# IXarea/LittleGAN

Hardware: AMD Instinct MI355X
Metric: 128x128 CelebA-shaped images/sec (G+D+Adj step) (higher is better)
Workload: dtype bf16; 1 GPU; C3: 128x128x3 synthetic CelebA, batch 256/GPU, bf16 MFMA conv/transposed-conv + Adjuster branch; global_batch=256, per_gpu_batch=256, image=128, cond_dim=40, parallelism=dp1, launch=eager launches

## Files before the change

### littlegan_amd/csrc/norm.hip

```cpp
#include "lg_common.h"
#include "philox.h"

#define LG_IN_EPS 1e-3f
#define LG_NSTAT 8

namespace {

constexpr int CHUNK = 4096;
constexpr int EW_UNR = 4;

__global__ __launch_bounds__(256) void stats_partial_kernel(const float* __restrict__ x, double* __restrict__ partial,
                                                            long long L, int nchunk, int pre_leaky, float alpha,
                                                            __bf16* __restrict__ x16out) {
  const int n = blockIdx.y, ch = blockIdx.x;
  const long long base = (long long)n * L + (long long)ch * CHUNK;
  const long long lim = L - (long long)ch * CHUNK;
  __shared__ double sred[32];
  f32x4 v[4];
  double s = 0.0;
  int cnt = 0;
#pragma unroll
  for (int q = 0; q < 4; ++q) {
    const int e = (q * 256 + threadIdx.x) * 4;
    v[q] = f32x4{0.f, 0.f, 0.f, 0.f};
// ... 183 lines not shown
   const long long lim = L - c0;
#pragma unroll
   for (int q = 0; q < 4; ++q) {
    const int e = (q * 256 + threadIdx.x) * 4;
    if (e < lim) {
      const f32x4 xv = *reinterpret_cast<const f32x4*>(x + base + e);
      const f32x4 gv = load_g4(g, base + e, g16);
      float q1 = 0.f, q2 = 0.f;
      float dm[4];
      if constexpr (DROP) drop_mult4(dc, (unsigned long long)(base + e) >> 2, dm);
#pragma unroll
      for (int k = 0; k < 4; ++k) {
        float xx = xv[k];
        if (pre_leaky) xx = lg_leaky(xx, alpha);
        const float c = (xx - mu) - mul;
        float dz = gv[k];
        if constexpr (DROP) dz = dz * dm[k];
        if (post_leaky) dz = (a * c + b > 0.f) ? dz : alpha * dz;
        q1 += dz;
        q2 += dz * c;
      }
      s1 += (double)q1;
      s2 += (double)q2;
    }
   }
  }
  double red[2] = {s1, s2};
  lg_block_sum_d<2>(red, sred);
  if (threadIdx.x == 0) {
    double* o = partial + ((long long)n * nchunk + blockIdx.x) * 2;
    o[0] = red[0]; o[1] = red[1];
  }
}

__global__ __launch_bounds__(256) void bwd_partial_kernel(const float* __restrict__ x, const void* __restrict__ g, int g16,
                                                          const float* __restrict__ stats, double* __restrict__ partial,
                                                          long long L, int nchunk, int pre_leaky, int post_leaky,
                                                          float alpha) {
  bwd_partial_body<false>(x, g, g16, stats, partial, L, nchunk, pre_leaky, post_leaky, alpha, DropK{}, Geo{blockDim.x, gridDim.x, gridDim.y});
}
__global__ __launch_bounds__(256) void bwd_partial_drop_kernel(const float* __restrict__ x, const void* __restrict__ g, int g16,
                                                               const float* __restrict__ stats, double* __restrict__ partial,
                                                               long long L, int nchunk, float alpha, DropK dk) {
  bwd_partial_body<true>(x, g, g16, stats, partial, L, nchunk, 0, 1, alpha, dk, Geo{blockDim.x, gridDim.x, gridDim.y});
}

__global__ __launch_bounds__(64) void bwd_final_kernel(const double* __restrict__ partial, const float* __restrict__ stats,
                                                       float* __restrict__ bstats, double* __restrict__ gsum,
                                                       long long L, int nchunk) {
  const int n = blockIdx.x, lane = threadIdx.x;
  const double* p = partial + (long long)n * nchunk * 2;
  double s1 = 0.0, s2 = 0.0;
  for (int i = lane; i < nchunk; i += 64) { s1 += p[i * 2]; s2 += p[i * 2 + 1]; }
  s1 = lg_wave_sum_d(s1); s2 = lg_wave_sum_d(s2);
  if (lane == 0) {
    const double sigma = (double)stats[(long long)n * LG_NSTAT + 1], s = sigma + (double)LG_IN_EPS;
    const double m1 = s1 / (double)L, m2 = s2 / (double)L / (s * sigma);
    const float m1h = (float)m1, m2h = (float)m2;
    bstats[n * 4] = m1h; bstats[n * 4 + 1] = m2h;
    bstats[n * 4 + 2] = (float)(m1 - (double)m1h); bstats[n * 4 + 3] = (float)(m2 - (double)m2h);
    gsum[n * 2] = s2 / s;
    gsum[n * 2 + 1] = s1;
  }
}

__global__ __launch_bounds__(64) void bwd_coef_kernel(const double* __restrict__ partial, const float* __restrict__ stats,
                                                      float* __restrict__ coef, long long L, int nchunk) {
  const int n = blockIdx.x, lane = threadIdx.x;
  const double* p = partial + (long long)n * nchunk * 2;
  double s1 = 0.0, s2 = 0.0;
  for (int i = lane; i < nchunk; i += 64) { s1 += p[i * 2]; s2 += p[i * 2 + 1]; }
  s1 = lg_wave_sum_d(s1); s2 = lg_wave_sum_d(s2);
  if (lane == 0) {
    const float* sp = stats + (long long)n * LG_NSTAT;
    const double sigma = (double)sp[1], s = sigma + (double)LG_IN_EPS;
    const double m1 = s1 / (double)L, m2 = s2 / (double)L / (s * sigma);
    const float m1h = (float)m1, m2h = (float)m2;
    float* o = coef + (long long)n * 8;
    o[0] = sp[0]; o[1] = sp[4]; o[2] = sp[2]; o[3] = sp[3];
    o[4] = m1h; o[5] = m2h; o[6] = (float)(m1 - (double)m1h); o[7] = (float)(m2 - (double)m2h);
  }
}

__global__ __launch_bounds__(256) void bwd_affine_grad_kernel(const double* __restrict__ gsum, float* __restrict__ dgamma,
                                                              float* __restrict__ dbeta, int B, int accumulate) {
  __shared__ double sg[256], sb[256];
  double g = 0.0, b = 0.0;
  for (int i = threadIdx.x; i < B; i += 256) { g += gsum[i * 2]; b += gsum[i * 2 + 1]; }
  sg[threadIdx.x] = g; sb[threadIdx.x] = b;
  __syncthreads();
  for (int o = 128; o > 0; o >>= 1) {
    if (threadIdx.x < o) { sg[threadIdx.x] += sg[threadIdx.x + o]; sb[threadIdx.x] += sb[threadIdx.x + o]; }
    __syncthreads();
  }
  if (threadIdx.x == 0) {
    dgamma[0] = (accumulate ? dgamma[0] : 0.f) + (float)sg[0];
    dbeta[0] = (accumulate ? dbeta[0] : 0.f) + (float)sb[0];
  }
}

template <bool DB, bool DROP>
__device__ __forceinline__ void bwd_apply_body(const float* __restrict__ x, const void* __restrict__ g, int g16,
                                               const float* __restrict__ stats, const float* __restrict__ bstats,
                                               float* __restrict__ dx, __bf16* __restrict__ dx16, long long L4,
                                               long long total4, int pre_leaky, int post_leaky, float alpha,
                                               float* __restrict__ colpart, int C4, const DropK& dk, const Geo ge) {
  const DropCtx dc = drop_begin<DROP>(dk);
  constexpr int UNR = DB ? 1 : EW_UNR;
  const unsigned stride = ge.gdx * ge.bdx * UNR, tot = (unsigned)total4, l4 = (unsigned)L4;
  f32x4 csum = {0.f, 0.f, 0.f, 0.f};
  const unsigned rb = blockIdx.x;
  const int ntrip = (int)(((unsigned long long)tot + stride - 1) / stride);
  for (int tr = 0; tr < ntrip; ++tr) {
   const unsigned long long i0l = (unsigned long long)tr * stride + rb * ge.bdx * UNR + threadIdx.x;
   if (i0l >= tot) continue;
   const unsigned i0 = (unsigned)i0l;
   f32x4 xs[UNR], gs[UNR];
#pragma unroll
   for (int u = 0; u < UNR; ++u) {
     const unsigned i = i0 + u * 256;
     if (i < tot) {
       xs[u] = lg_ld<NT_LOAD>(reinterpret_cast<const f32x4*>(x + (long long)i * 4));
       gs[u] = load_g4<NT_LOAD>(g, (long long)i * 4, g16);
     }
   }
#pragma unroll
   for (int u = 0; u < UNR; ++u) {
    const unsigned i = i0 + u * 256;
    if (i >= tot) break;
    const int n = (int)(i / l4);
    const float* sp = stats + (long long)n * LG_NSTAT;
    const float mu = sp[0], a = sp[2], b = sp[3], mul = sp[4];
    const float m1 = bstats[n * 4], m2 = bstats[n * 4 + 1], m1l = bstats[n * 4 + 2], m2l = bstats[n * 4 + 3];
    const f32x4 xv = xs[u], gv = gs[u];
    f32x4 o;
    float dm[4];
    if constexpr (DROP) drop_mult4(dc, i, dm);
#pragma unroll
    for (int k = 0; k < 4; ++k) {
      float xx = xv[k];
      if (pre_leaky) xx = lg_leaky(xx, alpha);
      const float c = (xx - mu) - mul;
      float dz = gv[k];
      if constexpr (DROP) dz = dz * dm[k];
      if (post_leaky) dz = (a * c + b > 0.f) ? dz : alpha * dz;
      float d = a * ((((dz - m1) - m1l) - c * m2) - c * m2l);
      if (pre_leaky) d = (xv[k] > 0.f) ? d : alpha * d;
      o[k] = d;
    }
    if (dx) *reinterpret_cast<f32x4*>(dx + (long long)i * 4) = o;
    if (dx16) {
      bf16x4 w;
      w[0] = (__bf16)o[0]; w[1] = (__bf16)o[1]; w[2] = (__bf16)o[2]; w[3] = (__bf16)o[3];
      *reinterpret_cast<bf16x4*>(dx16 + (long long)i * 4) = w;
    }
    if constexpr (DB) csum += o;
   }
  }
  if constexpr (DB) {
    __shared__ f32x4 sacc[256];
    sacc[threadIdx.x] = csum;
    __syncthreads();
    const int q = threadIdx.x;
    if (q < C4) {
      const int base = (int)(((long long)rb * 256) % C4);
      f32x4 t = {0.f, 0.f, 0.f, 0.f};
      for (int k = (q - base + C4) % C4; k < 256; k += C4) t += sacc[k];
      *reinterpret_cast<f32x4*>(colpart + ((long long)rb * C4 + q) * 4) = t;
    }
  }
}
template <bool DB>
__global__ __launch_bounds__(256) void bwd_apply_kernel(const float* __restrict__ x, const void* __restrict__ g, int g16,
                                                        const float* __restrict__ stats, const float* __restrict__ bstats,
                                                        float* __restrict__ dx, __bf16* __restrict__ dx16, long long L4,
                                                        long long total4, int pre_leaky, int post_leaky, float alpha,
                                                        float* __restrict__ colpart, int C4) {
  bwd_apply_body<DB, false>(x, g, g16, stats, bstats, dx, dx16, L4, total4, pre_leaky, post_leaky, alpha, colpart, C4, DropK{}, Geo{blockDim.x, gridDim.x, gridDim.y});
}
template <bool DB>
__global__ __launch_bounds__(256) void bwd_apply_drop_kernel(const float* __restrict__ x, const void* __restrict__ g, int g16,
// ... 253 lines not shown
                                                 long long total8, int pre_leaky, int post_leaky, float alpha,
                                                 float* __restrict__ colpart, int C8, const DropK& dk, const Geo ge) {
  const DropCtx dc = drop_begin<DROP>(dk);
  constexpr int UNR = DB ? DB_UNR : EW8_UNR;
  const unsigned tot = (unsigned)total8, l8 = (unsigned)L8;
  const unsigned ustep = DB ? ge.gdx * ge.bdx : 256u;
  const unsigned stride = DB ? ge.gdx * ge.bdx * UNR : ge.gdx * ge.bdx * UNR;
  const unsigned rb = ge.gdx - 1 - blockIdx.x;
  const unsigned first = DB ? rb * ge.bdx + threadIdx.x : rb * ge.bdx * UNR + threadIdx.x;
  f32x8 csum;
  csum.lo = f32x4{0.f, 0.f, 0.f, 0.f}; csum.hi = f32x4{0.f, 0.f, 0.f, 0.f};
  const int ntrip = (int)(((unsigned long long)tot + stride - 1) / stride);
  for (int tr = 0; tr < ntrip; ++tr) {
    const unsigned long long i0l = (unsigned long long)(ntrip - 1 - tr) * stride + first;
    if (i0l >= tot) continue;
    const unsigned i0 = (unsigned)i0l;
    f32x8 xs[UNR], gs[UNR];
#pragma unroll
    for (int u = 0; u < UNR; ++u) {
      const unsigned i = i0 + u * ustep;
      if (i < tot) { xs[u] = load8<true, NT_LOAD>(x, i); gs[u] = load8<G16, NT_LOAD>(g, i); }
    }
#pragma unroll
    for (int u = 0; u < UNR; ++u) {
      const unsigned i = i0 + u * ustep;
      if (i >= tot) break;
      const int n = (int)(i / l8);
      const float* sp = stats + (long long)n * LG_NSTAT;
      const float mu = sp[0], a = sp[2], b = sp[3], mul = sp[4];
      const float m1 = bstats[n * 4], m2 = bstats[n * 4 + 1], m1l = bstats[n * 4 + 2], m2l = bstats[n * 4 + 3];
      f32x8 o;
      float dm[8];
      if constexpr (DROP) drop_mult8(dc, i, dm);
#pragma unroll
      for (int k = 0; k < 8; ++k) {
        const float x0 = k < 4 ? xs[u].lo[k & 3] : xs[u].hi[k & 3];
        float xx = x0;
        if (pre_leaky) xx = lg_leaky(xx, alpha);
        const float c = (xx - mu) - mul;
        float dz = k < 4 ? gs[u].lo[k & 3] : gs[u].hi[k & 3];
        if constexpr (DROP) dz = dz * dm[k];
        if (post_leaky) dz = (a * c + b > 0.f) ? dz : alpha * dz;
        float d = a * ((((dz - m1) - m1l) - c * m2) - c * m2l);
        if (pre_leaky) d = (x0 > 0.f) ? d : alpha * d;
        if (k < 4) o.lo[k & 3] = d; else o.hi[k & 3] = d;
      }
      if (dx) store8_f32(dx, i, o);
      if (dx16) store8_bf16(dx16, i, o);
      if constexpr (DB) { csum.lo += o.lo; csum.hi += o.hi; }
    }
  }
  if constexpr (DB) {
    __shared__ f32x4 sacc[512];
    sacc[2 * threadIdx.x] = csum.lo; sacc[2 * threadIdx.x + 1] = csum.hi;
    __syncthreads();
    const int q = threadIdx.x;
    if (q < C8) {
      const int base = (int)(((long long)rb * 256) % C8);
      f32x4 tl = {0.f, 0.f, 0.f, 0.f}, th = {0.f, 0.f, 0.f, 0.f};
      for (int k = (q - base + C8) % C8; k < 256; k += C8) { tl += sacc[2 * k]; th += sacc[2 * k + 1]; }
      *reinterpret_cast<f32x4*>(colpart + ((long long)rb * C8 + q) * 8) = tl;
      *reinterpret_cast<f32x4*>(colpart + ((long long)rb * C8 + q) * 8 + 4) = th;
    }
  }
}

template <bool DB, bool G16>
__global__ __launch_bounds__(256) void bwd_apply16_kernel(const __bf16* __restrict__ x, const void* __restrict__ g,
                                                          const float* __restrict__ stats, const float* __restrict__ bstats,
                                                          float* __restrict__ dx, __bf16* __restrict__ dx16, long long L8,
                                                          long long total8, int pre_leaky, int post_leaky, float alpha,
                                                          float* __restrict__ colpart, int C8) {
  bwd_apply16_body<DB, G16, false>(x, g, stats, bstats, dx, dx16, L8, total8, pre_leaky, post_leaky, alpha, colpart, C8, DropK{}, Geo{blockDim.x, gridDim.x, gridDim.y});
}
template <bool DB, bool G16>
__global__ __launch_bounds__(256) void bwd_apply16_drop_kernel(const __bf16* __restrict__ x, const void* __restrict__ g,
                                                               const float* __restrict__ stats, const float* __restrict__ bstats,
                                                               float* __restrict__ dx, __bf16* __restrict__ dx16, long long L8,
                                                               long long total8, float alpha, float* __restrict__ colpart, int C8,
                                                               DropK dk) {
  bwd_apply16_body<DB, G16, true>(x, g, stats, bstats, dx, dx16, L8, total8, 0, 1, alpha, colpart, C8, dk, Geo{blockDim.x, gridDim.x, gridDim.y});
}

__global__ __launch_bounds__(256) void dropout_mask_kernel(unsigned char* __restrict__ keep, long long total8, DropK dk) {
  const DropCtx dc = drop_begin<true>(dk);
  for (long long i = (long long)blockIdx.x * 256 + threadIdx.x; i < total8; i += (long long)gridDim.x * 256) {
    float dm[8];
    drop_mult8(dc, (unsigned long long)i, dm);
    unsigned lo = 0, hi = 0;
#pragma unroll
    for (int k = 0; k < 4; ++k) { lo |= (dm[k] != 0.f ? 1u : 0u) << (8 * k); hi |= (dm[4 + k] != 0.f ? 1u : 0u) << (8 * k); }
    *reinterpret_cast<unsigned long long*>(keep + i * 8) = (unsigned long long)lo | ((unsigned long long)hi << 32);
  }
}

__global__ __launch_bounds__(1024) void colsum_final_kernel(const float* __restrict__ partial, float* __restrict__ db, int nb,
                                                            int C, int accumulate) {
  __shared__ float sr[64][17];
  const int cl = threadIdx.x & 15, gq = threadIdx.x >> 4;
  const int c = blockIdx.x * 16 + cl;
  float s = 0.f;
  if (c < C) {
    int k = gq;
    for (; k + 192 < nb; k += 256) {
      const float a = partial[(long long)k * C + c], b = partial[(long long)(k + 64) * C + c];
      const float e = partial[(long long)(k + 128) * C + c], f = partial[(long long)(k + 192) * C + c];
      s += (a + b) + (e + f);
    }
    for (; k < nb; k += 64) s += partial[(long long)k * C + c];
  }
  sr[gq][cl] = s;
  __syncthreads();
  if (gq == 0 && c < C) {
    float t = 0.f;
#pragma unroll
    for (int q = 0; q < 64; q += 4) t += (sr[q][cl] + sr[q + 1][cl]) + (sr[q + 2][cl] + sr[q + 3][cl]);
    db[c] = (accumulate ? db[c] : 0.f) + t;
  }
}

constexpr long long EW_MAX_BLOCKS = 8192;
extern "C" int lg_device_cus(void);
#define LG_RESIDENT_BLOCKS(kern)                                                                                       \
  ([]() -> long long {                                                                                                 \
    static long long r = 0;                                                                                            \
    if (!r) {                                                                                                          \
      int per_cu = 0;                                                                                                  \
      if (hipOccupancyMaxActiveBlocksPerMultiprocessor(&per_cu, kern, 256, 0) != hipSuccess || per_cu < 1) per_cu = 8; \
      r = (long long)per_cu * lg_device_cus();                                                                         \
    }                                                                                                                  \
    return r;                                                                                                          \
  }())
inline long long fit_rounds(long long nb, long long resident, long long hard, int unit) {
  if (nb > hard) nb = hard;
  if (nb > resident) nb = nb / resident * resident;
  nb = nb / unit * unit;
  return nb < unit ? unit : nb;
}
inline int nchunks(long long L) { return (int)((L + CHUNK - 1) / CHUNK); }
inline int ew_blocks(long long total4) {
  long long b = (total4 + 256 * EW_UNR - 1) / (256 * EW_UNR);
  return (int)(b < EW_MAX_BLOCKS ? (b > 0 ? b : 1) : EW_MAX_BLOCKS);
}
inline size_t part_bytes(int B, long long L) { return ((size_t)B * nchunks(L) * 3 * sizeof(double) + 255) / 256 * 256; }
inline size_t bst_bytes(int B) { return ((size_t)B * 4 * sizeof(float) + 255) / 256 * 256; }

int drop_args(const char* who, const long long* key, int call, int level, int r0, int B, long long L, float rate, DropK* dk) {
  LG_CHECK_ARG(key, "%s: null pointer (dropout key)", who);
  LG_CHECK_ARG(L > 0 && L % 8 == 0, "%s: dropout needs L %% 8 == 0 (one Philox block per 8 elements), got L=%lld", who, L);
  LG_CHECK_ARG(rate >= 0.f && rate < 1.f, "%s: dropout rate %g outside [0, 1)", who, (double)rate);
  LG_CHECK_ARG(call >= 0 && call <= 3, "%s: dropout call slot %d outside 0..3", who, call);
  LG_CHECK_ARG(level >= 1 && level <= 4, "%s: dropout level %d outside 1..4", who, level);
  LG_CHECK_ARG(r0 >= 0 && B > 0 && ((unsigned long long)r0 + (unsigned long long)B) * (unsigned long long)(L / 8) <= (1ull << 32),
               "%s: first row %d + %d rows of %lld elements leave the level's counter window", who, r0, B, L);
  const long long T = llrint((double)rate * 65536.0);
  LG_CHECK_ARG(T < 65536, "%s: dropout rate %g rounds to 1", who, (double)rate);
  dk->key = reinterpret_cast<const unsigned long long*>(key);
  dk->base = ((unsigned long long)call << 34) + ((unsigned long long)(level - 1) << 32) + (unsigned long long)r0 * (unsigned long long)(L / 8);
  dk->T = (unsigned)T;
  dk->scale = 65536.f / (float)(65536 - T);
  return LG_OK;
}

}

extern "C" int lg_instnorm_stats_stride(void) { return LG_NSTAT; }

extern "C" size_t lg_instnorm_workspace_bytes(int B, long long L) {
  const size_t gs = ((size_t)B * 2 * sizeof(double) + 255) / 256 * 256;
  return part_bytes(B, L) + bst_bytes(B) + gs;
}

extern "C" int lg_instnorm_leaky_stats_z16(const float* x, float* stats, const float* gamma, const float* beta,
                                           void* workspace, size_t ws_bytes, int B, long long L, int pre_leaky,
                                           float alpha, void* x16_out, void* stream);
extern "C" int lg_instnorm_leaky_stats(const float* x, float* stats, const float* gamma, const float* beta,
                                       void* workspace, size_t ws_bytes, int B, long long L, int pre_leaky,
                                       float alpha, void* stream) {
  return lg_instnorm_leaky_stats_z16(x, stats, gamma, beta, workspace, ws_bytes, B, L, pre_leaky, alpha, nullptr, stream);
}
extern "C" int lg_instnorm_leaky_stats_z16(const float* x, float* stats, const float* gamma, const float* beta,
                                           void* workspace, size_t ws_bytes, int B, long long L, int pre_leaky,
                                           float alpha, void* x16_out, void* stream) {
  LG_CHECK_ARG(x && stats && gamma && beta && workspace, "lg_instnorm_leaky_stats: null pointer");
  LG_CHECK_ARG(B > 0 && B <= 65535 && L > 0 && L % 4 == 0, "lg_instnorm_leaky_stats: bad shape B=%d L=%lld", B, L);
  LG_CHECK_ARG(ws_bytes >= lg_instnorm_workspace_bytes(B, L), "lg_instnorm_leaky_stats: workspace too small");
  hipStream_t st = (hipStream_t)stream;
  const int nc = nchunks(L);
  hipLaunchKernelGGL(stats_partial_kernel, dim3(nc, B), dim3(256), 0, st, x, (double*)workspace, L, nc, pre_leaky, alpha,
                     (__bf16*)x16_out);
  LG_CHECK_LAUNCH("lg_instnorm_leaky_stats(partial)");
  hipLaunchKernelGGL(stats_final_kernel, dim3(B), dim3(64), 0, st, (const double*)workspace, stats, gamma, beta, nc);
  LG_CHECK_LAUNCH("lg_instnorm_leaky_stats(final)");
  return LG_OK;
}

extern "C" int lg_instnorm_stats_finalize(const void* partials, int nparts, float* stats, const float* gamma,
                                          const float* beta, int B, void* stream) {
  LG_CHECK_ARG(partials && stats && gamma && beta && nparts > 0 && B > 0, "lg_instnorm_stats_finalize: bad arguments");
  hipLaunchKernelGGL(stats_final_kernel, dim3(B), dim3(64), 0, (hipStream_t)stream, (const double*)partials, stats, gamma,
                     beta, nparts);
  LG_CHECK_LAUNCH("lg_instnorm_stats_finalize");
  return LG_OK;
}

static int apply_impl(const float* x, const float* stats, const float* skip, float* y, void* y16, int B, long long L, int pre_leaky,
                      int post_leaky, float alpha, const DropK* dk, void* stream) {
  LG_CHECK_ARG(x && stats && (y || y16), "lg_instnorm_leaky_apply: null pointer");
  LG_CHECK_ARG(B > 0 && L > 0 && L % 4 == 0 && (long long)B * L / 4 < (1LL << 31), "lg_instnorm_leaky_apply: bad shape B=%d L=%lld", B, L);
  const long long total4 = (long long)B * L / 4;
  if (dk) {
    hipLaunchKernelGGL(apply_drop_kernel, dim3((int)fit_rounds(ew_blocks(total4), LG_RESIDENT_BLOCKS(apply_drop_kernel), EW_MAX_BLOCKS, 1)), dim3(256), 0,
                       (hipStream_t)stream, x, stats, y, (__bf16*)y16, L / 4, total4, alpha, *dk);
    LG_CHECK_LAUNCH("lg_instnorm_leaky_apply_drop");
    return LG_OK;
  }
  hipLaunchKernelGGL(apply_kernel, dim3((int)fit_rounds(ew_blocks(total4), LG_RESIDENT_BLOCKS(apply_kernel), EW_MAX_BLOCKS, 1)), dim3(256), 0, (hipStream_t)stream, x, stats, skip, y,
                     (__bf16*)y16, L / 4, total4, pre_leaky, post_leaky, alpha);
  LG_CHECK_LAUNCH("lg_instnorm_leaky_apply");
  return LG_OK;
}
extern "C" int lg_instnorm_leaky_apply(const float* x, const float* stats, const float* skip, float* y, void* y16, int B,
                                       long long L, int pre_leaky, int post_leaky, float alpha, void* stream) {
  return apply_impl(x, stats, skip, y, y16, B, L, pre_leaky, post_leaky, alpha, nullptr, stream);
}
extern "C" int lg_instnorm_leaky_apply_drop(const float* x, const float* stats, float* y, void* y16, int B, long long L, float alpha,
                                            const long long* key, int call, int level, int r0, float rate, void* stream) {
  DropK dk;
  if (int rc = drop_args("lg_instnorm_leaky_apply_drop", key, call, level, r0, B, L, rate, &dk)) return rc;
  return apply_impl(x, stats, nullptr, y, y16, B, L, 0, 1, alpha, &dk, stream);
}

constexpr int DB_MAX_BLOCKS = 2046;

extern "C" size_t lg_instnorm_bwd_db_workspace_bytes(int B, long long L, int C) {
  return lg_instnorm_workspace_bytes(B, L) + (size_t)DB_MAX_BLOCKS * (size_t)C * sizeof(float);
}

extern "C" int lg_instnorm_leaky_bwd_db(const float* x, const float* stats, const void* g, int g_is_bf16, float* dx, void* dx16,
                                        float* dgamma, float* dbeta, float* db, int C, void* workspace, size_t ws_bytes, int B,
                                        long long L, int pre_leaky, int post_leaky, float alpha, int accumulate, void* stream);

extern "C" int lg_instnorm_leaky_bwd(const float* x, const float* stats, const void* g, int g_is_bf16, float* dx, void* dx16,
                                     float* dgamma, float* dbeta, void* workspace, size_t ws_bytes, int B, long long L, int pre_leaky,
                                     int post_leaky, float alpha, int accumulate, void* stream) {
  return lg_instnorm_leaky_bwd_db(x, stats, g, g_is_bf16, dx, dx16, dgamma, dbeta, nullptr, 0, workspace, ws_bytes, B, L,
                                  pre_leaky, post_leaky, alpha, accumulate, stream);
}

static int bwd_impl(const float* x, const float* stats, const void* g, int g_is_bf16, float* dx, void* dx16,
                    float* dgamma, float* dbeta, float* db, int C, void* workspace, size_t ws_bytes, int B,
                    long long L, int pre_leaky, int post_leaky, float alpha, int accumulate, const DropK* dk, void* stream) {
  LG_CHECK_ARG(x && stats && g && (dx || dx16) && workspace, "lg_instnorm_leaky_bwd: null pointer");
  LG_CHECK_ARG(B > 0 && B <= 65535 && L > 0 && L % 4 == 0 && (long long)B * L / 4 < (1LL << 31),
               "lg_instnorm_leaky_bwd: bad shape B=%d L=%lld", B, L);
  LG_CHECK_ARG(ws_bytes >= lg_instnorm_workspace_bytes(B, L), "lg_instnorm_leaky_bwd: workspace too small");
  if (db) {
    LG_CHECK_ARG(C > 0 && C % 4 == 0 && C / 4 <= 256 && L % C == 0 && (256 % (C / 4) == 0 || 768 % (C / 4) == 0),
                 "lg_instnorm_leaky_bwd_db: unsupported channel count C=%d (L=%lld)", C, L);
    LG_CHECK_ARG(ws_bytes >= lg_instnorm_bwd_db_workspace_bytes(B, L, C), "lg_instnorm_leaky_bwd_db: workspace too small");
  }
  hipStream_t st = (hipStream_t)stream;
  int nc = 4096 / B;
  if (nc < 1) nc = 1;
  if (nc > nchunks(L)) nc = nchunks(L);
  char* ws = (char*)workspace;
  double* partial = (double*)ws;
  float* bstats = (float*)(ws + part_bytes(B, L));
  double* gsum = (double*)(ws + part_bytes(B, L) + bst_bytes(B));
  if (dk)
    hipLaunchKernelGGL(bwd_partial_drop_kernel, dim3(nc, B), dim3(256), 0, st, x, g, g_is_bf16, stats, partial, L, nc, alpha, *dk);
  else
    hipLaunchKernelGGL(bwd_partial_kernel, dim3(nc, B), dim3(256), 0, st, x, g, g_is_bf16, stats, partial, L, nc, pre_leaky,
                       post_leaky, alpha);
  LG_CHECK_LAUNCH("lg_instnorm_leaky_bwd(partial)");
  hipLaunchKernelGGL(bwd_final_kernel, dim3(B), dim3(64), 0, st, (const double*)partial, stats, bstats, gsum, L, nc);
  LG_CHECK_LAUNCH("lg_instnorm_leaky_bwd(final)");
  if (dgamma && dbeta) {
    hipLaunchKernelGGL(bwd_affine_grad_kernel, dim3(1), dim3(256), 0, st, (const double*)gsum, dgamma, dbeta, B,
                       accumulate);
    LG_CHECK_LAUNCH("lg_instnorm_leaky_bwd(affine)");
  }
  const long long total4 = (long long)B * L / 4;
  if (!db) {
    if (dk)
      hipLaunchKernelGGL(bwd_apply_drop_kernel<false>, dim3((int)fit_rounds(ew_blocks(total4), LG_RESIDENT_BLOCKS(bwd_apply_drop_kernel<false>), EW_MAX_BLOCKS, 1)), dim3(256), 0, st, x, g,
                         g_is_bf16, stats, (const float*)bstats, dx, (__bf16*)dx16, L / 4, total4, alpha, (float*)nullptr, 0, *dk);
    else
      hipLaunchKernelGGL(bwd_apply_kernel<false>, dim3((int)fit_rounds(ew_blocks(total4), LG_RESIDENT_BLOCKS(bwd_apply_kernel<false>), EW_MAX_BLOCKS, 1)), dim3(256), 0, st, x, g, g_is_bf16, stats,
                         (const float*)bstats, dx, (__bf16*)dx16, L / 4, total4, pre_leaky, post_leaky, alpha, nullptr, 0);
    LG_CHECK_LAUNCH("lg_instnorm_leaky_bwd(apply)");
    return LG_OK;
  }
  const int C4 = C / 4, unit = 256 % C4 == 0 ? 1 : 3;
  long long nb = fit_rounds((total4 + 255) / 256, LG_RESIDENT_BLOCKS(bwd_apply_kernel<true>), DB_MAX_BLOCKS, unit);
  float* colpart = (float*)(ws + lg_instnorm_workspace_bytes(B, L));
  if (dk)
    hipLaunchKernelGGL(bwd_apply_drop_kernel<true>, dim3((int)nb), dim3(256), 0, st, x, g, g_is_bf16, stats, (const float*)bstats, dx,
                       (__bf16*)dx16, L / 4, total4, alpha, colpart, C4, *dk);
  else
    hipLaunchKernelGGL(bwd_apply_kernel<true>, dim3((int)nb), dim3(256), 0, st, x, g, g_is_bf16, stats, (const float*)bstats, dx,
                       (__bf16*)dx16, L / 4, total4, pre_leaky, post_leaky, alpha, colpart, C4);
  LG_CHECK_LAUNCH("lg_instnorm_leaky_bwd_db(apply)");
  hipLaunchKernelGGL(colsum_final_kernel, dim3((C + 15) / 16), dim3(1024), 0, st, (const float*)colpart, db, (int)nb, C,
                     accumulate);
  LG_CHECK_LAUNCH("lg_instnorm_leaky_bwd_db(bias)");
  return LG_OK;
}
extern "C" int lg_instnorm_leaky_bwd_db(const float* x, const float* stats, const void* g, int g_is_bf16, float* dx, void* dx16,
                                        float* dgamma, float* dbeta, float* db, int C, void* workspace, size_t ws_bytes, int B,
                                        long long L, int pre_leaky, int post_leaky, float alpha, int accumulate, void* stream) {
  return bwd_impl(x, stats, g, g_is_bf16, dx, dx16, dgamma, dbeta, db, C, workspace, ws_bytes, B, L, pre_leaky, post_leaky, alpha,
                  accumulate, nullptr, stream);
}
extern "C" int lg_instnorm_leaky_bwd_drop(const float* x, const float* stats, const void* g, int g_is_bf16, float* dx, void* dx16,
                                          float* dgamma, float* dbeta, float* db, int C, void* workspace, size_t ws_bytes, int B,
// ... 54 lines not shown
  long long bps = (L8 + 256 * EW8_UNR * 4 - 1) / (256 * EW8_UNR * 4);
  if (bps * B > EW_MAX_BLOCKS) bps = EW_MAX_BLOCKS / B;
  if (bps < 1) bps = 1;
  hipStream_t st = (hipStream_t)stream;
  const dim3 grid((unsigned)bps, (unsigned)B);
  const __bf16* x = (const __bf16*)z16;
  const double* pr = (const double*)partials;
  if (dk)
    hipLaunchKernelGGL(apply16p_drop_kernel, grid, dim3(256), 0, st, x, pr, nparts, gamma, beta, stats, y, (__bf16*)y16, (unsigned)L8, alpha, *dk);
  else if (!skip)
    hipLaunchKernelGGL(apply16p_kernel<0>, grid, dim3(256), 0, st, x, pr, nparts, gamma, beta, stats, skip, y, (__bf16*)y16, (unsigned)L8, post_leaky, alpha);
  else if (!skip_is_bf16)
    hipLaunchKernelGGL(apply16p_kernel<1>, grid, dim3(256), 0, st, x, pr, nparts, gamma, beta, stats, skip, y, (__bf16*)y16, (unsigned)L8, post_leaky, alpha);
  else
    hipLaunchKernelGGL(apply16p_kernel<2>, grid, dim3(256), 0, st, x, pr, nparts, gamma, beta, stats, skip, y, (__bf16*)y16, (unsigned)L8, post_leaky, alpha);
  LG_CHECK_LAUNCH("lg_instnorm_leaky_apply_z16_p");
  return LG_OK;
}
extern "C" int lg_instnorm_leaky_apply_z16_p(const void* z16, const void* partials, int nparts, const float* gamma, const float* beta,
                                             float* stats, const void* skip, int skip_is_bf16, float* y, void* y16, int B,
                                             long long L, int post_leaky, float alpha, void* stream) {
  return apply16p_impl(z16, partials, nparts, gamma, beta, stats, skip, skip_is_bf16, y, y16, B, L, post_leaky, alpha, nullptr, stream);
}
extern "C" int lg_instnorm_leaky_apply_z16_p_drop(const void* z16, const void* partials, int nparts, const float* gamma, const float* beta,
                                                  float* stats, float* y, void* y16, int B, long long L, float alpha,
                                                  const long long* key, int call, int level, int r0, float rate, void* stream) {
  DropK dk;
  if (int rc = drop_args("lg_instnorm_leaky_apply_z16_p_drop", key, call, level, r0, B, L, rate, &dk)) return rc;
  return apply16p_impl(z16, partials, nparts, gamma, beta, stats, nullptr, 0, y, y16, B, L, 1, alpha, &dk, stream);
}

extern "C" int lg_instnorm_leaky_bwd_z16_p(const void* z16, const float* stats, const void* g, int g_is_bf16, float* dx,
                                           void* dx16, float* dgamma, float* dbeta, float* db, int C, const void* partials,
                                           int nparts_in, void* workspace, size_t ws_bytes, int B, long long L, int pre_leaky,
                                           int post_leaky, float alpha, int accumulate, void* stream);
extern "C" int lg_instnorm_leaky_bwd_z16(const void* z16, const float* stats, const void* g, int g_is_bf16, float* dx,
                                         void* dx16, float* dgamma, float* dbeta, float* db, int C, void* workspace,
                                         size_t ws_bytes, int B, long long L, int pre_leaky, int post_leaky, float alpha,
                                         int accumulate, void* stream) {
  return lg_instnorm_leaky_bwd_z16_p(z16, stats, g, g_is_bf16, dx, dx16, dgamma, dbeta, db, C, nullptr, 0, workspace, ws_bytes, B, L,
                                     pre_leaky, post_leaky, alpha, accumulate, stream);
}
static int bwd16_impl(const void* z16, const float* stats, const void* g, int g_is_bf16, float* dx, void* dx16, float* dgamma, float* dbeta,
                      float* db, int C, const void* partials, int nparts_in, void* workspace, size_t ws_bytes, int B, long long L,
                      int pre_leaky, int post_leaky, float alpha, int accumulate, const DropK* dk, void* stream) {
  LG_CHECK_ARG(z16 && stats && g && (dx || dx16) && workspace, "lg_instnorm_leaky_bwd_z16: null pointer");
  LG_CHECK_ARG(!(dk && partials && nparts_in > 0 && dk->T != 0), "lg_instnorm_leaky_bwd_z16_drop: fused partial sums know no dropout mask");
  LG_CHECK_ARG(B > 0 && B <= 65535 && L > 0 && L % 8 == 0 && (long long)B * L / 8 < (1LL << 31),
               "lg_instnorm_leaky_bwd_z16: bad shape B=%d L=%lld", B, L);
  LG_CHECK_ARG(ws_bytes >= lg_instnorm_workspace_bytes(B, L), "lg_instnorm_leaky_bwd_z16: workspace too small");
  LG_CHECK_ARG(!(partials && nparts_in > 0) || (pre_leaky == 0 && post_leaky == 1),
               "lg_instnorm_leaky_bwd_z16_p: fused partial sums exist for pre_leaky=0, post_leaky=1 only (got %d, %d)", pre_leaky, post_leaky);
  if (db) {
    LG_CHECK_ARG(C > 0 && C % 8 == 0 && C / 8 <= 256 && L % C == 0 && (256 % (C / 8) == 0 || 768 % (C / 8) == 0),
                 "lg_instnorm_leaky_bwd_z16: unsupported channel count C=%d (L=%lld)", C, L);
    LG_CHECK_ARG(ws_bytes >= lg_instnorm_bwd_db_workspace_bytes(B, L, C), "lg_instnorm_leaky_bwd_z16: workspace too small");
  }
  hipStream_t st = (hipStream_t)stream;
  const __bf16* x = (const __bf16*)z16;
  int nc = 4096 / B;
  if (nc < 1) nc = 1;
  const int nch8 = (int)((L + 2 * CHUNK - 1) / (2 * CHUNK));
  if (nc > nch8) nc = nch8;
  char* ws = (char*)workspace;
  double* partial = (double*)ws;
  float* bstats = (float*)(ws + part_bytes(B, L));
  double* gsum = (double*)(ws + part_bytes(B, L) + bst_bytes(B));
  if (partials && nparts_in > 0) {
    partial = (double*)partials;
    nc = nparts_in;
  } else {
    if (dk && g_is_bf16)
      hipLaunchKernelGGL(bwd_partial16_drop_kernel<true>, dim3(nc, B), dim3(256), 0, st, x, g, stats, partial, L, nc, alpha, *dk);
    else if (dk)
      hipLaunchKernelGGL(bwd_partial16_drop_kernel<false>, dim3(nc, B), dim3(256), 0, st, x, g, stats, partial, L, nc, alpha, *dk);
    else if (g_is_bf16)
      hipLaunchKernelGGL(bwd_partial16_kernel<true>, dim3(nc, B), dim3(256), 0, st, x, g, stats, partial, L, nc, pre_leaky,
                         post_leaky, alpha);
    else
      hipLaunchKernelGGL(bwd_partial16_kernel<false>, dim3(nc, B), dim3(256), 0, st, x, g, stats, partial, L, nc, pre_leaky,
                         post_leaky, alpha);
    LG_CHECK_LAUNCH("lg_instnorm_leaky_bwd_z16(partial)");
  }
  hipLaunchKernelGGL(bwd_final_kernel, dim3(B), dim3(64), 0, st, (const double*)partial, stats, bstats, gsum, L, nc);
  LG_CHECK_LAUNCH("lg_instnorm_leaky_bwd_z16(final)");
  if (dgamma && dbeta) {
    hipLaunchKernelGGL(bwd_affine_grad_kernel, dim3(1), dim3(256), 0, st, (const double*)gsum, dgamma, dbeta, B, accumulate);
    LG_CHECK_LAUNCH("lg_instnorm_leaky_bwd_z16(affine)");
  }
  const long long total8 = (long long)B * L / 8;
  if (!db) {
    long long nb = (total8 + 256 * EW8_UNR - 1) / (256 * EW8_UNR);
    if (dk)
      nb = fit_rounds(nb, g_is_bf16 ? LG_RESIDENT_BLOCKS((bwd_apply16_drop_kernel<false, true>)) : LG_RESIDENT_BLOCKS((bwd_apply16_drop_kernel<false, false>)), EW_MAX_BLOCKS, 1);
    else
      nb = fit_rounds(nb, g_is_bf16 ? LG_RESIDENT_BLOCKS((bwd_apply16_kernel<false, true>)) : LG_RESIDENT_BLOCKS((bwd_apply16_kernel<false, false>)), EW_MAX_BLOCKS, 1);
    if (dk && g_is_bf16)
      hipLaunchKernelGGL((bwd_apply16_drop_kernel<false, true>), dim3((int)nb), dim3(256), 0, st, x, g, stats, (const float*)bstats, dx,
                         (__bf16*)dx16, L / 8, total8, alpha, (float*)nullptr, 0, *dk);
    else if (dk)
      hipLaunchKernelGGL((bwd_apply16_drop_kernel<false, false>), dim3((int)nb), dim3(256), 0, st, x, g, stats, (const float*)bstats, dx,
                         (__bf16*)dx16, L / 8, total8, alpha, (float*)nullptr, 0, *dk);
    else if (g_is_bf16)
      hipLaunchKernelGGL((bwd_apply16_kernel<false, true>), dim3((int)nb), dim3(256), 0, st, x, g, stats, (const float*)bstats, dx,
                         (__bf16*)dx16, L / 8, total8, pre_leaky, post_leaky, alpha, (float*)nullptr, 0);
    else
      hipLaunchKernelGGL((bwd_apply16_kernel<false, false>), dim3((int)nb), dim3(256), 0, st, x, g, stats, (const float*)bstats, dx,
                         (__bf16*)dx16, L / 8, total8, pre_leaky, post_leaky, alpha, (float*)nullptr, 0);
    LG_CHECK_LAUNCH("lg_instnorm_leaky_bwd_z16(apply)");
    return LG_OK;
  }
  const int C8 = C / 8, unit = 256 % C8 == 0 ? 1 : 3;
  long long nb = (total8 + 511) / 512;
  nb = fit_rounds(nb, g_is_bf16 ? LG_RESIDENT_BLOCKS((bwd_apply16_kernel<true, true>)) : LG_RESIDENT_BLOCKS((bwd_apply16_kernel<true, false>)), DB_MAX_BLOCKS, unit);
  float* colpart = (float*)(ws + lg_instnorm_workspace_bytes(B, L));
  if (dk && g_is_bf16)
    hipLaunchKernelGGL((bwd_apply16_drop_kernel<true, true>), dim3((int)nb), dim3(256), 0, st, x, g, stats, (const float*)bstats, dx,
                       (__bf16*)dx16, L / 8, total8, alpha, colpart, C8, *dk);
  else if (dk)
    hipLaunchKernelGGL((bwd_apply16_drop_kernel<true, false>), dim3((int)nb), dim3(256), 0, st, x, g, stats, (const float*)bstats, dx,
                       (__bf16*)dx16, L / 8, total8, alpha, colpart, C8, *dk);
  else if (g_is_bf16)
    hipLaunchKernelGGL((bwd_apply16_kernel<true, true>), dim3((int)nb), dim3(256), 0, st, x, g, stats, (const float*)bstats, dx,
                       (__bf16*)dx16, L / 8, total8, pre_leaky, post_leaky, alpha, colpart, C8);
  else
    hipLaunchKernelGGL((bwd_apply16_kernel<true, false>), dim3((int)nb), dim3(256), 0, st, x, g, stats, (const float*)bstats, dx,
                       (__bf16*)dx16, L / 8, total8, pre_leaky, post_leaky, alpha, colpart, C8);
  LG_CHECK_LAUNCH("lg_instnorm_leaky_bwd_z16(apply+bias)");
  hipLaunchKernelGGL(colsum_final_kernel, dim3((C + 15) / 16), dim3(1024), 0, st, (const float*)colpart, db, (int)nb, C,
                     accumulate);
  LG_CHECK_LAUNCH("lg_instnorm_leaky_bwd_z16(bias)");
  return LG_OK;
}
extern "C" int lg_instnorm_leaky_bwd_z16_p(const void* z16, const float* stats, const void* g, int g_is_bf16, float* dx,
                                           void* dx16, float* dgamma, float* dbeta, float* db, int C, const void* partials,
                                           int nparts_in, void* workspace, size_t ws_bytes, int B, long long L, int pre_leaky,
                                           int post_leaky, float alpha, int accumulate, void* stream) {
  return bwd16_impl(z16, stats, g, g_is_bf16, dx, dx16, dgamma, dbeta, db, C, partials, nparts_in, workspace, ws_bytes, B, L, pre_leaky,
                    post_leaky, alpha, accumulate, nullptr, stream);
}
extern "C" int lg_instnorm_leaky_bwd_z16_drop(const void* z16, const float* stats, const void* g, int g_is_bf16, float* dx, void* dx16,
                                              float* dgamma, float* dbeta, float* db, int C, const void* partials, int nparts_in,
                                              void* workspace, size_t ws_bytes, int B, long long L, float alpha, int accumulate,
                                              const long long* key, int call, int level, int r0, float rate, void* stream) {
  DropK dk;
  if (int rc = drop_args("lg_instnorm_leaky_bwd_z16_drop", key, call, level, r0, B, L, rate, &dk)) return rc;
  return bwd16_impl(z16, stats, g, g_is_bf16, dx, dx16, dgamma, dbeta, db, C, partials, nparts_in, workspace, ws_bytes, B, L, 0, 1, alpha,
                    accumulate, &dk, stream);
}

__global__ void dropout_key_kernel(unsigned long long* __restrict__ key, unsigned long long seed, unsigned long long key_offset) {
  if (threadIdx.x == 0) { key[0] = seed; key[1] = key_offset; }
}
extern "C" int lg_dropout_key(long long* key, unsigned long long seed, unsigned long long key_offset, void* stream) {
  LG_CHECK_ARG(key && ((uintptr_t)key & 7) == 0, "lg_dropout_key: null or misaligned pointer");
  hipLaunchKernelGGL(dropout_key_kernel, dim3(1), dim3(64), 0, (hipStream_t)stream, reinterpret_cast<unsigned long long*>(key), seed, key_offset);
  LG_CHECK_LAUNCH("lg_dropout_key");
  return LG_OK;
}

extern "C" int lg_dropout_mask(const long long* key, int call, int level, int r0, int B, long long L, float rate, unsigned char* keep,
                               void* stream) {
  LG_CHECK_ARG(keep, "lg_dropout_mask: null pointer");
  LG_CHECK_ARG(((uintptr_t)keep & 7) == 0, "lg_dropout_mask: keep must be 8-byte aligned (8 decisions per store)");
  LG_CHECK_ARG(B > 0 && L > 0 && (long long)B * L / 8 < (1LL << 31), "lg_dropout_mask: bad shape B=%d L=%lld", B, L);
  DropK dk;
  if (int rc = drop_args("lg_dropout_mask", key, call, level, r0, B, L, rate, &dk)) return rc;
  const long long total8 = (long long)B * L / 8;
  long long nb = (total8 + 255) / 256;
  if (nb > EW_MAX_BLOCKS) nb = EW_MAX_BLOCKS;
  hipLaunchKernelGGL(dropout_mask_kernel, dim3((int)nb), dim3(256), 0, (hipStream_t)stream, keep, total8, dk);
  LG_CHECK_LAUNCH("lg_dropout_mask");
  return LG_OK;
// ... 10 lines not shown
```

Baseline: 23750 images/sec.

## Fuse instance-norm backward finalization into per-sample apply kernel and merge bias/affine reductions

Adds a per-sample 2D-grid backward apply kernel. Each block reduces the chunk partials for its sample in one wavefront and derives the coefficients itself, which removes the separate bwd_final launch. The bias column-sum and the affine gamma/beta reduction are merged into one kernel launch. Block traversal is reversed, likely so that recently written data is reused from cache. The cost is redundant partial reductions in every block and a more complex grid-sizing heuristic, with a fallback to the old path when the grid does not fit.

```diff
diff --git a/littlegan_amd/csrc/norm.hip b/littlegan_amd/csrc/norm.hip
--- a/littlegan_amd/csrc/norm.hip
+++ b/littlegan_amd/csrc/norm.hip
@@ -289,12 +289,14 @@
   }
 }
 
-__global__ __launch_bounds__(256) void bwd_affine_grad_kernel(const double* __restrict__ gsum, float* __restrict__ dgamma,
-                                                              float* __restrict__ dbeta, int B, int accumulate) {
+__device__ __forceinline__ void bwd_affine_grad_body(const double* __restrict__ gsum, float* __restrict__ dgamma,
+                                                     float* __restrict__ dbeta, int B, int accumulate) {
   __shared__ double sg[256], sb[256];
-  double g = 0.0, b = 0.0;
-  for (int i = threadIdx.x; i < B; i += 256) { g += gsum[i * 2]; b += gsum[i * 2 + 1]; }
-  sg[threadIdx.x] = g; sb[threadIdx.x] = b;
+  if (threadIdx.x < 256) {
+    double g = 0.0, b = 0.0;
+    for (int i = threadIdx.x; i < B; i += 256) { g += gsum[i * 2]; b += gsum[i * 2 + 1]; }
+    sg[threadIdx.x] = g; sb[threadIdx.x] = b;
+  }
   __syncthreads();
   for (int o = 128; o > 0; o >>= 1) {
     if (threadIdx.x < o) { sg[threadIdx.x] += sg[threadIdx.x + o]; sb[threadIdx.x] += sb[threadIdx.x + o]; }
@@ -304,6 +306,10 @@
     dgamma[0] = (accumulate ? dgamma[0] : 0.f) + (float)sg[0];
     dbeta[0] = (accumulate ? dbeta[0] : 0.f) + (float)sb[0];
   }
+}
+__global__ __launch_bounds__(256) void bwd_affine_grad_kernel(const double* __restrict__ gsum, float* __restrict__ dgamma,
+                                                              float* __restrict__ dbeta, int B, int accumulate) {
+  bwd_affine_grad_body(gsum, dgamma, dbeta, B, accumulate);
 }
 
 template <bool DB, bool DROP>
@@ -723,6 +729,118 @@
   bwd_apply16_body<DB, G16, true>(x, g, stats, bstats, dx, dx16, L8, total8, 0, 1, alpha, colpart, C8, dk, Geo{blockDim.x, gridDim.x, gridDim.y});
 }
 
+template <bool DB, bool G16, bool DROP>
+__device__ __forceinline__ void bwd_apply16p_body(const __bf16* __restrict__ x, const void* __restrict__ g,
+                                                  const float* __restrict__ stats, const double* __restrict__ partial, int nchunk,
+                                                  float* __restrict__ bstats, double* __restrict__ gsum,
+                                                  float* __restrict__ dx, __bf16* __restrict__ dx16, unsigned L8, int pre_leaky,
+                                                  int post_leaky, float alpha, float* __restrict__ colpart, int C8, const DropK& dk,
+                                                  const Geo ge) {
+  const DropCtx dc = drop_begin<DROP>(dk);
+  __shared__ float sco[8];
+  const int n = (int)(ge.gdy - 1 - blockIdx.y);
+  const unsigned bx = ge.gdx - 1 - blockIdx.x;
+  if (threadIdx.x < 64) {
+    const int lane = threadIdx.x;
+    const double* p = partial + (long long)n * nchunk * 2;
+    double s1 = 0.0, s2 = 0.0;
+    for (int i = lane; i < nchunk; i += 64) { s1 += p[i * 2]; s2 += p[i * 2 + 1]; }
+    s1 = lg_wave_sum_d(s1); s2 = lg_wave_sum_d(s2);
+    if (lane == 0) {
+      const float* sp = stats + (long long)n * LG_NSTAT;
+      const double L = (double)((long long)L8 * 8);
+      const double sigma = (double)sp[1], s = sigma + (double)LG_IN_EPS;
+      const double m1 = s1 / L, m2 = s2 / L / (s * sigma);
+      const float m1h = (float)m1, m2h = (float)m2;
+      const float m1l = (float)(m1 - (double)m1h), m2l = (float)(m2 - (double)m2h);
+      sco[0] = sp[0]; sco[1] = sp[2]; sco[2] = sp[3]; sco[3] = sp[4];
+      sco[4] = m1h; sco[5] = m2h; sco[6] = m1l; sco[7] = m2l;
+      if (bx == 0) {
+        bstats[n * 4] = m1h; bstats[n * 4 + 1] = m2h; bstats[n * 4 + 2] = m1l; bstats[n * 4 + 3] = m2l;
+        gsum[n * 2] = s2 / s;
+        gsum[n * 2 + 1] = s1;
+      }
+    }
+  }
+  __syncthreads();
+  const float mu = sco[0], a = sco[1], b = sco[2], mul = sco[3];
+  const float m1 = sco[4], m2 = sco[5], m1l = sco[6], m2l = sco[7];
+  constexpr int UNR = DB ? DB_UNR : EW8_UNR;
+  const long long base = (long long)n * L8;
+  const unsigned ustep = DB ? ge.gdx * ge.bdx : 256u;
+  const unsigned stride = ge.gdx * ge.bdx * UNR;
+  const unsigned first = DB ? bx * ge.bdx + threadIdx.x : bx * ge.bdx * UNR + threadIdx.x;
+  f32x8 csum;
+  csum.lo = f32x4{0.f, 0.f, 0.f, 0.f}; csum.hi = f32x4{0.f, 0.f, 0.f, 0.f};
+  const int ntrip = (int)(((unsigned long long)L8 + stride - 1) / stride);
+  for (int tr = 0; tr < ntrip; ++tr) {
+    const unsigned long long i0l = (unsigned long long)(ntrip - 1 - tr) * stride + first;
+    if (i0l >= L8) continue;
+    const unsigned i0 = (unsigned)i0l;
+    f32x8 xs[UNR], gs[UNR];
+#pragma unroll
+    for (int u = 0; u < UNR; ++u) {
+      const unsigned long long i = (unsigned long long)i0 + (unsigned long long)u * ustep;
+      if (i < L8) { xs[u] = load8<true, NT_LOAD>(x, base + (long long)i); gs[u] = load8<G16, NT_LOAD>(g, base + (long long)i); }
+    }
+#pragma unroll
+    for (int u = 0; u < UNR; ++u) {
+      const unsigned long long i = (unsigned long long)i0 + (unsigned long long)u * ustep;
+      if (i >= L8) break;
+      f32x8 o;
+      float dm[8];
+      if constexpr (DROP) drop_mult8(dc, (unsigned long long)(base + (long long)i), dm);
+#pragma unroll
+      for (int k = 0; k < 8; ++k) {
+        const float x0 = k < 4 ? xs[u].lo[k & 3] : xs[u].hi[k & 3];
+        float xx = x0;
+        if (pre_leaky) xx = lg_leaky(xx, alpha);
+        const float c = (xx - mu) - mul;
+        float dz = k < 4 ? gs[u].lo[k & 3] : gs[u].hi[k & 3];
+        if constexpr (DROP) dz = dz * dm[k];
+        if (post_leaky) dz = (a * c + b > 0.f) ? dz : alpha * dz;
+        float d = a * ((((dz - m1) - m1l) - c * m2) - c * m2l);
+        if (pre_leaky) d = (x0 > 0.f) ? d : alpha * d;
+        if (k < 4) o.lo[k & 3] = d; else o.hi[k & 3] = d;
+      }
+      if (dx) store8_f32(dx, base + (long long)i, o);
+      if (dx16) store8_bf16(dx16, base + (long long)i, o);
+      if constexpr (DB) { csum.lo += o.lo; csum.hi += o.hi; }
+    }
+  }
+  if constexpr (DB) {
+    __shared__ f32x4 sacc[512];
+    sacc[2 * threadIdx.x] = csum.lo; sacc[2 * threadIdx.x + 1] = csum.hi;
+    __syncthreads();
+    const int q = threadIdx.x;
+    if (q < C8) {
+      const long long row = (long long)n * ge.gdx + bx;
+      const int cb = (int)(((long long)bx * 256) % C8);
+      f32x4 tl = {0.f, 0.f, 0.f, 0.f}, th = {0.f, 0.f, 0.f, 0.f};
+      for (int k = (q - cb + C8) % C8; k < 256; k += C8) { tl += sacc[2 * k]; th += sacc[2 * k + 1]; }
+      *reinterpret_cast<f32x4*>(colpart + (row * C8 + q) * 8) = tl;
+      *reinterpret_cast<f32x4*>(colpart + (row * C8 + q) * 8 + 4) = th;
+    }
+  }
+}
+
+template <bool DB, bool G16>
+__global__ __launch_bounds__(256) void bwd_apply16p_kernel(const __bf16* __restrict__ x, const void* __restrict__ g,
+                                                           const float* __restrict__ stats, const double* __restrict__ partial, int nchunk,
+                                                           float* __restrict__ bstats, double* __restrict__ gsum,
+                                                           float* __restrict__ dx, __bf16* __restrict__ dx16, unsigned L8, int pre_leaky,
+                                                           int post_leaky, float alpha, float* __restrict__ colpart, int C8) {
+  bwd_apply16p_body<DB, G16, false>(x, g, stats, partial, nchunk, bstats, gsum, dx, dx16, L8, pre_leaky, post_leaky, alpha, colpart, C8, DropK{}, Geo{blockDim.x, gridDim.x, gridDim.y});
+}
+template <bool DB, bool G16>
+__global__ __launch_bounds__(256) void bwd_apply16p_drop_kernel(const __bf16* __restrict__ x, const void* __restrict__ g,
+                                                                const float* __restrict__ stats, const double* __restrict__ partial, int nchunk,
+                                                                float* __restrict__ bstats, double* __restrict__ gsum,
+                                                                float* __restrict__ dx, __bf16* __restrict__ dx16, unsigned L8, float alpha,
+                                                                float* __restrict__ colpart, int C8, DropK dk) {
+  bwd_apply16p_body<DB, G16, true>(x, g, stats, partial, nchunk, bstats, gsum, dx, dx16, L8, 0, 1, alpha, colpart, C8, dk, Geo{blockDim.x, gridDim.x, gridDim.y});
+}
+
 __global__ __launch_bounds__(256) void dropout_mask_kernel(unsigned char* __restrict__ keep, long long total8, DropK dk) {
   const DropCtx dc = drop_begin<true>(dk);
   for (long long i = (long long)blockIdx.x * 256 + threadIdx.x; i < total8; i += (long long)gridDim.x * 256) {
@@ -735,8 +853,8 @@
   }
 }
 
-__global__ __launch_bounds__(1024) void colsum_final_kernel(const float* __restrict__ partial, float* __restrict__ db, int nb,
-                                                            int C, int accumulate) {
+__device__ __forceinline__ void colsum_final_body(const float* __restrict__ partial, float* __restrict__ db, int nb,
+                                                  int C, int accumulate) {
   __shared__ float sr[64][17];
   const int cl = threadIdx.x & 15, gq = threadIdx.x >> 4;
   const int c = blockIdx.x * 16 + cl;
@@ -759,8 +877,19 @@
     db[c] = (accumulate ? db[c] : 0.f) + t;
   }
 }
+__global__ __launch_bounds__(1024) void colsum_final_kernel(const float* __restrict__ partial, float* __restrict__ db, int nb,
+                                                            int C, int accumulate) {
+  colsum_final_body(partial, db, nb, C, accumulate);
+}
+__global__ __launch_bounds__(1024) void colsum_affine_final_kernel(const float* __restrict__ partial, float* __restrict__ db, int nb,
+                                                                   int C, const double* __restrict__ gsum, float* __restrict__ dgamma,
+                                                                   float* __restrict__ dbeta, int B, int accumulate) {
+  if (blockIdx.x + 1 == gridDim.x) bwd_affine_grad_body(gsum, dgamma, dbeta, B, accumulate);
+  else colsum_final_body(partial, db, nb, C, accumulate);
+}
 
 constexpr long long EW_MAX_BLOCKS = 8192;
+constexpr int DB_MAX_BLOCKS = 2046;
 extern "C" int lg_device_cus(void);
 #define LG_RESIDENT_BLOCKS(kern)                                                                                       \
   ([]() -> long long {                                                                                                 \
@@ -803,6 +932,45 @@
   return LG_OK;
 }
 
+template <bool DB, bool G16>
+long long bwd16p_gdx(int B, long long L8, int unit) {
+  if (L8 < 256) return 0;
+  const long long resident = LG_RESIDENT_BLOCKS((bwd_apply16p_kernel<DB, G16>));
+  const long long bt = (L8 + 511) / 512, hard = DB ? DB_MAX_BLOCKS : EW_MAX_BLOCKS;
+  long long want = bt;
+  if (!DB) {
+    long long round1 = (resident + B - 1) / B;
+    if (round1 > bt) round1 = bt;
+    want = (bt + 3) / 4;
+    if (want < round1) want = round1;
+  }
+  const long long nbt = fit_rounds(want * B, resident, hard, unit * B);
+  if (nbt > hard) return 0;
+  return nbt / B;
+}
+const char* bwd16_name(bool aligned, bool db, bool g16, bool drop) {
+  static const char* const names[2][2][2][2] = {
+      {{{"bwd_apply16_kernel<false,false>", "bwd_apply16_kernel<false,true>"}, {"bwd_apply16_kernel<true,false>", "bwd_apply16_kernel<true,true>"}},
+       {{"bwd_apply16_drop_kernel<false,false>", "bwd_apply16_drop_kernel<false,true>"},
+        {"bwd_apply16_drop_kernel<true,false>", "bwd_apply16_drop_kernel<true,true>"}}},
+      {{{"bwd_apply16p_kernel<false,false>", "bwd_apply16p_kernel<false,true>"}, {"bwd_apply16p_kernel<true,false>", "bwd_apply16p_kernel<true,true>"}},
+       {{"bwd_apply16p_drop_kernel<false,false>", "bwd_apply16p_drop_kernel<false,true>"},
+        {"bwd_apply16p_drop_kernel<true,false>", "bwd_apply16p_drop_kernel<true,true>"}}}};
+  return names[aligned][drop][db][g16];
+}
+template <bool DB, bool G16>
+void launch_bwd16p(dim3 grid, hipStream_t st, const DropK* dk, const __bf16* x, const void* g, const float* stats, const double* partial,
+                   int nc, float* bstats, double* gsum, float* dx, __bf16* dx16, unsigned L8, int pre_leaky, int post_leaky, float alpha,
+                   float* colpart, int C8) {
+  if (dk)
+    hipLaunchKernelGGL((bwd_apply16p_drop_kernel<DB, G16>), grid, dim3(256), 0, st, x, g, stats, partial, nc, bstats, gsum, dx, dx16, L8,
+                       alpha, colpart, C8, *dk);
+  else
+    hipLaunchKernelGGL((bwd_apply16p_kernel<DB, G16>), grid, dim3(256), 0, st, x, g, stats, partial, nc, bstats, gsum, dx, dx16, L8,
+                       pre_leaky, post_leaky, alpha, colpart, C8);
+  lg_note_kernel(bwd16_name(true, DB, G16, dk != nullptr));
+}
+
 }
 
 extern "C" int lg_instnorm_stats_stride(void) { return LG_NSTAT; }
@@ -871,8 +1039,6 @@
   if (int rc = drop_args("lg_instnorm_leaky_apply_drop", key, call, level, r0, B, L, rate, &dk)) return rc;
   return apply_impl(x, stats, nullptr, y, y16, B, L, 0, 1, alpha, &dk, stream);
 }
-
-constexpr int DB_MAX_BLOCKS = 2046;
 
 extern "C" size_t lg_instnorm_bwd_db_workspace_bytes(int B, long long L, int C) {
   return lg_instnorm_workspace_bytes(B, L) + (size_t)DB_MAX_BLOCKS * (size_t)C * sizeof(float);
@@ -1093,13 +1259,45 @@
                          post_leaky, alpha);
     LG_CHECK_LAUNCH("lg_instnorm_leaky_bwd_z16(partial)");
   }
+  const long long total8 = (long long)B * L / 8;
+  const int unit16 = db ? (256 % (C / 8) == 0 ? 1 : 3) : 1;
+  const long long gdx = g_is_bf16 ? (db ? bwd16p_gdx<true, true>(B, L / 8, unit16) : bwd16p_gdx<false, true>(B, L / 8, unit16))
+                                  : (db ? bwd16p_gdx<true, false>(B, L / 8, unit16) : bwd16p_gdx<false, false>(B, L / 8, unit16));
+  if (gdx > 0) {
+    float* colpart = db ? (float*)(ws + lg_instnorm_workspace_bytes(B, L)) : nullptr;
+    const dim3 grid((unsigned)gdx, (unsigned)B);
+    const unsigned L8 = (unsigned)(L / 8);
+    const int C8 = db ? C / 8 : 0;
+    if (db && g_is_bf16)
+      launch_bwd16p<true, true>(grid, st, dk, x, g, stats, partial, nc, bstats, gsum, dx, (__bf16*)dx16, L8, pre_leaky, post_leaky, alpha, colpart, C8);
+    else if (db)
+      launch_bwd16p<true, false>(grid, st, dk, x, g, stats, partial, nc, bstats, gsum, dx, (__bf16*)dx16, L8, pre_leaky, post_leaky, alpha, colpart, C8);
+    else if (g_is_bf16)
+      launch_bwd16p<false, true>(grid, st, dk, x, g, stats, partial, nc, bstats, gsum, dx, (__bf16*)dx16, L8, pre_leaky, post_leaky, alpha, colpart, C8);
+    else
+      launch_bwd16p<false, false>(grid, st, dk, x, g, stats, partial, nc, bstats, gsum, dx, (__bf16*)dx16, L8, pre_leaky, post_leaky, alpha, colpart, C8);
+    LG_CHECK_LAUNCH("lg_instnorm_leaky_bwd_z16(apply_p)");
+    if (db && dgamma && dbeta) {
+      hipLaunchKernelGGL(colsum_affine_final_kernel, dim3((C + 15) / 16 + 1), dim3(1024), 0, st, (const float*)colpart, db,
+                         (int)(gdx * B), C, (const double*)gsum, dgamma, dbeta, B, accumulate);
+      LG_CHECK_LAUNCH("lg_instnorm_leaky_bwd_z16(bias+affine)");
+    } else if (db) {
+      hipLaunchKernelGGL(colsum_final_kernel, dim3((C + 15) / 16), dim3(1024), 0, st, (const float*)colpart, db, (int)(gdx * B), C,
+                         accumulate);
+      LG_CHECK_LAUNCH("lg_instnorm_leaky_bwd_z16(bias)");
+    } else if (dgamma && dbeta) {
+      hipLaunchKernelGGL(bwd_affine_grad_kernel, dim3(1), dim3(256), 0, st, (const double*)gsum, dgamma, dbeta, B, accumulate);
+      LG_CHECK_LAUNCH("lg_instnorm_leaky_bwd_z16(affine)");
+    }
+    return LG_OK;
+  }
+  lg_note_kernel(bwd16_name(false, db != nullptr, g_is_bf16 != 0, dk != nullptr));
   hipLaunchKernelGGL(bwd_final_kernel, dim3(B), dim3(64), 0, st, (const double*)partial, stats, bstats, gsum, L, nc);
   LG_CHECK_LAUNCH("lg_instnorm_leaky_bwd_z16(final)");
   if (dgamma && dbeta) {
     hipLaunchKernelGGL(bwd_affine_grad_kernel, dim3(1), dim3(256), 0, st, (const double*)gsum, dgamma, dbeta, B, accumulate);
     LG_CHECK_LAUNCH("lg_instnorm_leaky_bwd_z16(affine)");
   }
-  const long long total8 = (long long)B * L / 8;
   if (!db) {
     long long nb = (total8 + 256 * EW8_UNR - 1) / (256 * EW8_UNR);
     if (dk)
```

Result: no change. 23980 images/sec, median of 6 (+1.0%).
